# raulmur/ORB_SLAM2

Hardware: AMD Instinct MI355X
Metric: frames/s ORB extract+match, 1241x376 gray, 2000 kpts, 8 lvls (higher is better)
Workload: dtype u8

## Files before the change

### orb_slam2_amd/csrc/orbhip_kernels_extract.hip

```cpp
#include "orbhip_internal.h"
#include <type_traits>

#define WAVE 64

__device__ __forceinline__ bool xcd_frame_map(int nb, int nframes, int& tile, int& frame)
{
    const int id = blockIdx.x;
    if (nframes == 1) { tile = id; frame = 0; return true; }
    if (nframes < 8) { tile = id / nframes; frame = id - tile * nframes; return true; }
    const int j = id >> 3, fg = j / nb;
    tile = j - fg * nb; frame = fg * 8 + (id & 7);
    return frame < nframes;
}
static inline unsigned xcd_grid(int nb, int nframes) { return nframes < 8 ? (unsigned)nb * (unsigned)nframes : (unsigned)nb * 8u * (unsigned)((nframes + 7) / 8); }

typedef unsigned short pku16 __attribute__((vector_size(4)));
typedef short pki16 __attribute__((vector_size(4)));
typedef unsigned u32_unaligned __attribute__((aligned(1)));
#define ORBHIP_GLOBAL __attribute__((address_space(1)))
template <typename T> __device__ __forceinline__ ORBHIP_GLOBAL T* uniform_ptr(T* p)
{
    const unsigned long long a = (unsigned long long)p;
    const unsigned lo = (unsigned)__builtin_amdgcn_readfirstlane((int)(unsigned)a), hi = (unsigned)__builtin_amdgcn_readfirstlane((int)(unsigned)(a >> 32));
    return (ORBHIP_GLOBAL T*)(((unsigned long long)hi << 32) | lo);
// ... 263 lines not shown
    int tile, frame;
    if (!xcd_frame_map(gx * gyn, P.nframes, tile, frame)) return;
    frame += P.frame0;
    __shared__ unsigned s_t0[PYR_SROWS * PYR_SDW], s_t1[PYR_SROWS * PYR_SDW];
    const int tid = threadIdx.y * 64 + threadIdx.x, wv = __builtin_amdgcn_readfirstlane((int)threadIdx.y);
    const int tx = tile % gx;
    int ty = (tile / gx) * nt;
    const int tyend = min(ty + nt, gy);
    PyrStep st;
    st.S.src = level_src(P, frame, level - 1, st.S.spitch);
    st.T = pyr_dma_issue(P, g, tx, ty, tid, s_t0, st.S);
    const PyrGroup G = P.xgrp[g.xgrp_off + min(tx * (PYR_TW / 4) + (int)threadIdx.x, (g.w - 1) >> 2)];
    for (; ty < tyend; ty += 2) {
        pyr_step(P, g, tx, ty, tyend, frame, tid, threadIdx.x, wv, G, s_t0, s_t1, st);
        if (ty + 1 < tyend) pyr_step(P, g, tx, ty + 1, tyend, frame, tid, threadIdx.x, wv, G, s_t1, s_t0, st);
    }
}

__global__ __launch_bounds__(256) void k_pyramid_level_direct(ExtractParams P, int level)
{
    const LevelGeom g = P.geom[level];
    const int gx = (g.w + PYR_TW - 1) / PYR_TW, gy = (g.h + PYR_TH - 1) / PYR_TH;
    int tile, frame;
    if (!xcd_frame_map(gx * gy, P.nframes, tile, frame)) return;
    frame += P.frame0;
    const int x4 = (tile % gx) * PYR_TW + threadIdx.x * 4, ytop = (tile / gx) * PYR_TH + threadIdx.y * PYR_RPT;
    if (x4 >= g.w) return;
    int spitch; const uint8_t* src = level_src(P, frame, level - 1, spitch);
    pyr_rows(g, P.xtab + g.xtab_off, P.ytab + g.ytab_off, src, spitch, 0, x4, ytop, P.pyr + (long long)frame * P.plane_frame_bytes + g.plane_off + x4);
}

__device__ __forceinline__ int qt_wave_incl_scan(int v, int lane);
#define PC_T 256
#define PC_GIT 3
#define PC_YIT 2
#define PC_RIT 16
struct PcLevel { int w, src_h, pitch, plane_off, xgrp_off, ytab_off, goff, yoff, x0, x1, y0, y1; unsigned rcp; };
__global__ __launch_bounds__(PC_T) void k_pyramid_cascade(ExtractParams P)
{
    HIP_DYNAMIC_SHARED(unsigned char, pc_lds)
    __shared__ PcLevel s_lv[ORBHIP_MAX_LEVELS];
    int tile, frame;
    if (!xcd_frame_map(P.pc_ntx * P.pc_nty, P.nframes, tile, frame)) return;
    frame += P.frame0;
    const int tid = (int)threadIdx.x, L = P.nlevels;
    const int ty = tile / P.pc_ntx, tx = tile - ty * P.pc_ntx;
    if (tid < 64) {
        const int l = min(tid, L - 1);
        const LevelGeom g = P.geom[l];
        const short2 a = P.pc_xr[l * P.pc_ntx + tx], b = P.pc_yr[l * P.pc_nty + ty];
        const int ng = ((a.y - a.x) >> 2) + 1;
        const int nx = (tid >= 1 && tid < L) ? ng : 0, ny = (tid >= 1 && tid < L) ? b.y - b.x + 1 : 0;
        const int go = qt_wave_incl_scan(nx, tid) - nx, yo = qt_wave_incl_scan(ny, tid) - ny;
        if (tid < L) s_lv[tid] = PcLevel{g.w, g.src_h, g.pitch, g.plane_off, g.xgrp_off, g.ytab_off, go, yo, a.x, a.y, b.x, b.y, 0xffffffffu / (unsigned)ng + 1u};
        if (tid == L - 1) { s_lv[0].goff = go + nx; s_lv[0].yoff = yo + ny; }
    }
    __syncthreads();
    uint4* const s_grp = reinterpret_cast<uint4*>(pc_lds + P.pc_buf0 + P.pc_buf1);
    int2* const s_yt = reinterpret_cast<int2*>(s_grp + 3 * P.pc_xcap);
    {
        const int gtot = s_lv[0].goff, ytot = s_lv[0].yoff;
        int goffs[ORBHIP_MAX_LEVELS], yoffs[ORBHIP_MAX_LEVELS];
#pragma unroll
        for (int l = 0; l < ORBHIP_MAX_LEVELS; l++) { goffs[l] = s_lv[min(l, L - 1)].goff; yoffs[l] = s_lv[min(l, L - 1)].yoff; }
        uint4 gv[PC_GIT]; int2 yv[PC_YIT]; unsigned rv[PC_RIT];
#pragma unroll
        for (int k = 0; k < PC_GIT; k++) {
            const int i = min(tid + PC_T * k, 3 * gtot - 1), e = i / 3, piece = i - 3 * e;
            int l = 1;
#pragma unroll
            for (int q = 2; q < ORBHIP_MAX_LEVELS; q++) if (q < L && e >= goffs[q]) l = q;
            const PcLevel& v = s_lv[l];
            gv[k] = reinterpret_cast<const uint4*>(P.xgrp + v.xgrp_off + (v.x0 >> 2) + (e - v.goff))[piece];
        }
#pragma unroll
        for (int k = 0; k < PC_YIT; k++) {
            const int i = min(tid + PC_T * k, ytot - 1);
            int l = 1;
#pragma unroll
            for (int q = 2; q < ORBHIP_MAX_LEVELS; q++) if (q < L && i >= yoffs[q]) l = q;
            const PcLevel& v = s_lv[l];
            yv[k] = P.ytab[v.ytab_off + v.y0 + i - v.yoff];
        }
        const PcLevel R = s_lv[0];
        int spitch; const uint8_t* src = level_src(P, frame, 0, spitch);
        const int ng = ((R.x1 - R.x0) >> 2) + 1, n0 = ng * (R.y1 - R.y0 + 1);
#pragma unroll
        for (int k = 0; k < PC_RIT; k++) {
            const int i = min(tid + PC_T * k, n0 - 1);
            const int r = ng == 1 ? i : (int)__umulhi((unsigned)i, R.rcp), g4 = i - r * ng, x = R.x0 + 4 * g4;
            const uint8_t* p = src + (long long)(R.y0 + r) * spitch + x;
            unsigned w;
            if (x + 3 < R.w) w = *reinterpret_cast<const u32_unaligned*>(p);
            else { w = 0; for (int q = 0; q < 4; q++) if (x + q < R.w) w |= (unsigned)p[q] << (8 * q); }
            rv[k] = w;
        }
#pragma unroll
        for (int k = 0; k < PC_GIT; k++) if (tid + PC_T * k < 3 * gtot) s_grp[tid + PC_T * k] = gv[k];
#pragma unroll
        for (int k = 0; k < PC_YIT; k++) if (tid + PC_T * k < ytot) s_yt[tid + PC_T * k] = yv[k];
#pragma unroll
        for (int k = 0; k < PC_RIT; k++) if (tid + PC_T * k < n0) reinterpret_cast<unsigned*>(pc_lds)[tid + PC_T * k] = rv[k];
    }
    __syncthreads();
    for (int l = 1; l < L; l++) {
        const PcLevel R = s_lv[l], S = s_lv[l - 1];
        const int ng = ((R.x1 - R.x0) >> 2) + 1, rows = R.y1 - R.y0 + 1, spd = ((S.x1 - S.x0) >> 2) + 1;
        const unsigned* sb = reinterpret_cast<const unsigned*>(pc_lds + ((l & 1) ? 0 : P.pc_buf0));
        unsigned* db = reinterpret_cast<unsigned*>(pc_lds + ((l & 1) ? P.pc_buf0 : 0));
        const PyrGroup* grp = reinterpret_cast<const PyrGroup*>(s_grp) + R.goff; const int2* yt = s_yt + R.yoff;
        uint8_t* gdst = P.pyr + (long long)frame * P.plane_frame_bytes + R.plane_off;
        const bool keep = l + 1 < L;
        for (int i = tid; i < ng * rows; i += PC_T) {
            const int gy = ng == 1 ? i : (int)__umulhi((unsigned)i, R.rcp), g4 = i - gy * ng, y = R.y0 + gy, x4 = R.x0 + 4 * g4;
            const PyrGroup G = grp[g4];
            const int2 ye = yt[gy];
            const unsigned b0s = (unsigned)ye.y << 16, b1s = (unsigned)ye.y & 0xffff0000u;
            const int ra = min(max(ye.x, 0), R.src_h - 1) - S.y0, rb = min(max(ye.x + 1, 0), R.src_h - 1) - S.y0;
            const unsigned sh = (unsigned)G.sx0 & 3u;
            const unsigned* colp = sb + ((G.sx0 - S.x0) >> 2);
            unsigned h0[4], h1[4];
            pyr_hrow(colp + ra * spd, sh, G, h0);
            pyr_hrow(colp + rb * spd, sh, G, h1);
            unsigned out = 0;
#pragma unroll
            for (int k = 0; k < 4; k++) out |= ((__umulhi(b0s, h0[k]) + __umulhi(b1s, h1[k]) + 2u) >> 2) << (8 * k);
            out &= x4 + 4 <= R.w ? 0xffffffffu : (0xffffffffu >> (8 * (x4 + 4 - R.w)));
            if (keep) db[i] = out;
            *reinterpret_cast<unsigned*>(gdst + (long long)y * R.pitch + x4) = out;
        }
        lds_barrier();
    }
}
void orbhip_launch_pyramid_cascade(const ExtractParams& P, int nframes, hipStream_t s)
{
    ExtractParams Q = P; Q.nframes = nframes;
    const size_t lds = (size_t)P.pc_buf0 + P.pc_buf1 + (size_t)P.pc_xcap * sizeof(PyrGroup) + (size_t)P.pc_ycap * sizeof(int2);
    hipLaunchKernelGGL(k_pyramid_cascade, dim3(xcd_grid(P.pc_ntx * P.pc_nty, nframes), 1, 1), dim3(PC_T, 1, 1), lds, s, Q);
}

bool orbhip_pyramid_tile_fits(int src_cols_per_tile, int src_rows_per_tile) { return ((src_cols_per_tile + 3) >> 2) + 1 <= PYR_SDW && src_rows_per_tile <= PYR_SROWS; }
int orbhip_pyramid_tile_dwords() { return PYR_SDW; }
int orbhip_blur_mfma_tile_w() { return BM_COLS * BM_BLOCKS; }
int orbhip_blur_mfma_tile_h() { return BM_ROWS; }
int orbhip_pyramid_tile_w() { return PYR_TW; }
int orbhip_pyramid_tile_h() { return PYR_TH; }

void orbhip_launch_pyramid_level(const ExtractParams& P, int level, int w, int h, int mode, int nframes, hipStream_t s)
{
    ExtractParams Q = P; Q.nframes = nframes;
    dim3 grid(xcd_grid(((w + PYR_TW - 1) / PYR_TW) * ((h + PYR_TH - 1) / PYR_TH), nframes), 1, 1), block(64, 4, 1);
    static const int nt_env = getenv("ORBHIP_PYR_NT") ? atoi(getenv("ORBHIP_PYR_NT")) : 0;
    const int nt = nt_env > 0 ? nt_env : nframes >= 384 ? 4 : nframes <= 8 ? 1 : 2;
    const int gyn = (((h + PYR_TH - 1) / PYR_TH) + nt - 1) / nt;
    if (mode == 2) hipLaunchKernelGGL(k_pyramid_level_g, dim3(xcd_grid(((w + PYR_TW - 1) / PYR_TW) * gyn, nframes), 1, 1), block, 0, s, Q, level, nt);
    else if (mode == 1) hipLaunchKernelGGL(k_pyramid_level, grid, block, 0, s, Q, level);
    else hipLaunchKernelGGL(k_pyramid_level_direct, grid, block, 0, s, Q, level);
}

struct GrayParams {
    const uint8_t* src; long long src_frame_stride; int src_row_stride;
    uint8_t* dst; long long dst_frame_stride; int dst_pitch;
    int w, h, channels, k0, k2;
};
__device__ __forceinline__ uint32_t gray14(uint32_t c0, uint32_t c1, uint32_t c2, int k0, int k2)
{
    return (c0 * (uint32_t)k0 + c1 * 9617u + c2 * (uint32_t)k2 + 8192u) >> 14;
}
__global__ __launch_bounds__(256) void k_to_gray(GrayParams G)
{
    const int x = (blockIdx.x * 256 + threadIdx.x) * 4, y = blockIdx.y, f = blockIdx.z;
    if (x >= G.w) return;
    const uint8_t* srow = G.src + (long long)f * G.src_frame_stride + (long long)y * G.src_row_stride + (long long)x * G.channels;
    uint8_t* drow = G.dst + (long long)f * G.dst_frame_stride + (long long)y * G.dst_pitch + x;
    const bool whole = x + 4 <= G.w, aligned = (((uintptr_t)srow) & 3) == 0;
    if (whole && aligned) {
        const uint32_t* s4 = (const uint32_t*)srow;
        uint32_t g0, g1, g2, g3;
        if (G.channels == 3) {
            const uint32_t a = s4[0], b = s4[1], c = s4[2];
            g0 = gray14(a & 255, (a >> 8) & 255, (a >> 16) & 255, G.k0, G.k2);
            g1 = gray14(a >> 24, b & 255, (b >> 8) & 255, G.k0, G.k2);
            g2 = gray14((b >> 16) & 255, b >> 24, c & 255, G.k0, G.k2);
            g3 = gray14((c >> 8) & 255, (c >> 16) & 255, c >> 24, G.k0, G.k2);
        } else {
            const uint32_t a = s4[0], b = s4[1], c = s4[2], d = s4[3];
            g0 = gray14(a & 255, (a >> 8) & 255, (a >> 16) & 255, G.k0, G.k2);
            g1 = gray14(b & 255, (b >> 8) & 255, (b >> 16) & 255, G.k0, G.k2);
            g2 = gray14(c & 255, (c >> 8) & 255, (c >> 16) & 255, G.k0, G.k2);
            g3 = gray14(d & 255, (d >> 8) & 255, (d >> 16) & 255, G.k0, G.k2);
        }
        *(uint32_t*)drow = g0 | (g1 << 8) | (g2 << 16) | (g3 << 24);
    } else {
        const int n = min(4, G.w - x);
        for (int i = 0; i < n; i++) {
            const uint8_t* p = srow + i * G.channels;
            drow[i] = (uint8_t)gray14(p[0], p[1], p[2], G.k0, G.k2);
        }
    }
}
void orbhip_launch_to_gray(const uint8_t* src, long long src_frame_stride, int src_row_stride, uint8_t* dst, long long dst_frame_stride,
                           int dst_pitch, int w, int h, int channels, bool rgb_order, int nframes, hipStream_t s)
{
    GrayParams G{src, src_frame_stride, src_row_stride, dst, dst_frame_stride, dst_pitch, w, h, channels,
                 rgb_order ? 4899 : 1868, rgb_order ? 1868 : 4899};
    dim3 grid((w + 1023) / 1024, h, nframes), block(256, 1, 1);
    hipLaunchKernelGGL(k_to_gray, grid, block, 0, s, G);
}

#define BLUR_TW 128
#define BLUR_TH 32
#define BLUR_SROW 144
__device__ __forceinline__ int reflect101_clamped(int p, int len)
{
    if (p < 0) p = -p; else if (p >= len) p = 2 * (len - 1) - p;
    return min(max(p, 0), len - 1);
}
struct BlurK { float k0, k1, k2, k3; unsigned dot_lo, dot_hi; };
#define BLUR_SDW (BLUR_SROW / 4)
#define BLUR_SROWS (BLUR_TH + 6)
__global__ __launch_bounds__(256) void k_blur(ExtractParams P, BlurK K)
{
    int tile, frame;
    if (!xcd_frame_map(P.nblur_tiles, P.nframes, tile, frame)) return;
    frame += P.frame0;
    const TileDesc t = P.blur_tiles[tile];
    const int tid = threadIdx.x;
    const LevelGeom g = P.geom[t.level];
    int spitch; const uint8_t* src = level_src(P, frame, t.level, spitch);
    __shared__ unsigned s_src[BLUR_SROWS * BLUR_SDW];
    __shared__ float4 s_h[BLUR_SROWS * (BLUR_TW / 4)];
    const bool aligned = ((((unsigned long long)src) | (unsigned long long)spitch) & 3ull) == 0;
    {
        const int wave = __builtin_amdgcn_readfirstlane(tid >> 6), lane = tid & 63;
        const int gx = t.x0 - 4 + 4 * lane;
        const bool act = lane < 34, edge = act && !(aligned && gx >= 0 && gx + 3 < g.w);
        unsigned v[10];
#pragma unroll
        for (int j = 0; j < 10; j++) {
            const uint8_t* row = src + (long long)reflect101_clamped(t.y0 - 3 + wave + 4 * j, g.h) * spitch + (t.x0 - 4);
            v[j] = (act && !edge) ? *reinterpret_cast<const unsigned*>(row + (unsigned)(4 * lane)) : 0u;
        }
        if (edge) {
            const int x0r = reflect101_clamped(gx, g.w), x1r = reflect101_clamped(gx + 1, g.w), x2r = reflect101_clamped(gx + 2, g.w), x3r = reflect101_clamped(gx + 3, g.w);
#pragma unroll
            for (int j = 0; j < 10; j++) {
                const uint8_t* row = src + (long long)reflect101_clamped(t.y0 - 3 + wave + 4 * j, g.h) * spitch;
                v[j] = (unsigned)row[x0r] | ((unsigned)row[x1r] << 8) | ((unsigned)row[x2r] << 16) | ((unsigned)row[x3r] << 24);
            }
        }
#pragma unroll
        for (int j = 0; j < 10; j++) {
            const int r = wave + 4 * j;
            if (act && r < BLUR_SROWS) s_src[r * BLUR_SDW + lane] = v[j];
        }
    }
    __syncthreads();
    for (int i = tid; i < BLUR_SROWS * 32; i += 256) {
        const int r = i >> 5, q = i & 31;
        const unsigned* p = &s_src[r * BLUR_SDW + q];
        const unsigned w0 = p[0], w1 = p[1], w2 = p[2];
        float4 o;
        o.x = (float)__builtin_amdgcn_udot4(__builtin_amdgcn_alignbyte(w1, w0, 1), K.dot_lo, __builtin_amdgcn_udot4(__builtin_amdgcn_alignbyte(w2, w1, 1), K.dot_hi, 0u, false), false);
        o.y = (float)__builtin_amdgcn_udot4(__builtin_amdgcn_alignbyte(w1, w0, 2), K.dot_lo, __builtin_amdgcn_udot4(__builtin_amdgcn_alignbyte(w2, w1, 2), K.dot_hi, 0u, false), false);
        o.z = (float)__builtin_amdgcn_udot4(__builtin_amdgcn_alignbyte(w1, w0, 3), K.dot_lo, __builtin_amdgcn_udot4(__builtin_amdgcn_alignbyte(w2, w1, 3), K.dot_hi, 0u, false), false);
        o.w = (float)__builtin_amdgcn_udot4(w1, K.dot_lo, __builtin_amdgcn_udot4(w2, K.dot_hi, 0u, false), false);
        s_h[r * (BLUR_TW / 4) + q] = o;
    }
    __syncthreads();
    const int q = tid & 31, rg = tid >> 5;
    const int gx = t.x0 + 4 * q;
    if (gx >= g.w) return;
    float h[10][4];
#pragma unroll
    for (int r = 0; r < 10; r++) { const float4 v = s_h[(4 * rg + r) * (BLUR_TW / 4) + q]; h[r][0] = v.x; h[r][1] = v.y; h[r][2] = v.z; h[r][3] = v.w; }
    const bool half_even = P.blur_round_mode == 1 && gx < (g.w & ~3);
    uint8_t* dstbase = P.blur + (long long)frame * P.plane_frame_bytes + g.plane_off + gx;
    auto strip = [&](auto he) {
#pragma unroll
        for (int r = 0; r < 4; r++) {
            const int gy = t.y0 + 4 * rg + r;
            if (gy >= g.h) break;
            unsigned out = 0;
#pragma unroll
            for (int k = 0; k < 4; k++) {
                float sum = K.k0 * h[r + 3][k];
                sum = __builtin_fmaf(K.k1, h[r + 2][k] + h[r + 4][k], sum);
                sum = __builtin_fmaf(K.k2, h[r + 1][k] + h[r + 5][k], sum);
                sum = __builtin_fmaf(K.k3, h[r][k] + h[r + 6][k], sum);
                const float v = decltype(he)::value ? sum * (1.0f / 65536.0f) : __builtin_floorf(__builtin_fmaf(sum, 1.0f / 65536.0f, 0.5f));
                out = __builtin_amdgcn_cvt_pk_u8_f32(v, (unsigned)k, out);
            }
            *reinterpret_cast<unsigned*>(dstbase + (long long)gy * g.pitch) = out;
        }
    };
    if (half_even) strip(std::true_type{}); else strip(std::false_type{});
}

typedef int v4i __attribute__((vector_size(16)));
typedef int v2i __attribute__((vector_size(8)));
typedef int v16i __attribute__((vector_size(64)));
#define BM_IN_DW 68
#define BM_OUT_DW 57
struct BlurTile { TileDesc t; LevelGeom g; const uint8_t* src; int spitch; };
__device__ __forceinline__ BlurTile blur_tile(const ExtractParams& P, int frame, int tile)
{
    BlurTile T; T.t = P.blur_tiles[tile]; T.g = P.geom[T.t.level]; T.src = level_src(P, frame, T.t.level, T.spitch);
    return T;
}
__device__ __forceinline__ void blur_issue(const BlurTile& T, int wave, int lane, unsigned* s_in)
{
    const LevelGeom& g = T.g; const int x0 = T.t.x0, y0 = T.t.y0, spitch = T.spitch; const uint8_t* src = T.src;
    const int w4 = g.w & ~3;
    const int c0 = x0 - 4 + 4 * lane;
    const unsigned coff = (unsigned)min(max(c0, 0), w4 - 4);
#pragma unroll
    for (int r = 0; r < 8; r++) {
        const int row = 8 * wave + r;
        const ORBHIP_GLOBAL uint8_t* rp = uniform_ptr(src + (long long)reflect101_clamped(y0 - 3 + row, g.h) * spitch);
        lds_dma_dword(rp + coff, reinterpret_cast<uint8_t*>(s_in + row * BM_IN_DW));
    }
}
__device__ __forceinline__ void blur_fix(const BlurTile& T, int wave, int lane, unsigned* s_in)
{
    const LevelGeom& g = T.g; const int x0 = T.t.x0, y0 = T.t.y0, spitch = T.spitch; const uint8_t* src = T.src;
    const int w4 = g.w & ~3;
    const bool fix_left = x0 == 0, fix_right = x0 + 252 > w4;
    if (fix_left || fix_right) {
        const int rr = lane >> 3, slot = lane & 7, row = 8 * wave + rr;
        const int cfix = slot == 0 ? -4 : w4 + 4 * (slot - 1);
        const int dw = (cfix - (x0 - 4)) >> 2;
        const bool act = (slot == 0 ? fix_left : (slot <= 2 && fix_right)) && dw >= 0 && dw < 64;
        if (act) {
            const uint8_t* rowp = src + (long long)reflect101_clamped(y0 - 3 + row, g.h) * spitch;
            unsigned wv = 0;
#pragma unroll
            for (int b = 0; b < 4; b++) wv |= (unsigned)rowp[reflect101_clamped(cfix + b, g.w)] << (8 * b);
            s_in[row * BM_IN_DW + dw] = wv;
        }
    }
}
__device__ __forceinline__ void blur_compute(const ExtractParams& P, const BlurTile& T, int wave, int lane, const unsigned* s_in, unsigned* s_out, const unsigned* s_band)
{
    const LevelGeom& g = T.g; const int x0 = T.t.x0;
    const int w4 = g.w & ~3;
    const int i = lane & 31, h = lane >> 5;
    const v4i HB1 = *reinterpret_cast<const v4i*>(s_band + 4 * lane), HB2 = *reinterpret_cast<const v4i*>(s_band + 256 + 4 * lane), VB = *reinterpret_cast<const v4i*>(s_band + 512 + 4 * lane);
    const v16i zero = {0, 0, 0, 0, 0, 0, 0, 0, 0, 0, 0, 0, 0, 0, 0, 0};
    const int he_limit = P.blur_round_mode == 1 ? w4 : 0;
    const float kbias = (float)(257 * 128 * 257) * (1.0f / 65536.0f);
#pragma unroll 1
    for (int c = wave; c < BM_BLOCKS; c += 4) {
        const int xb = x0 + 32 * c;
        if (xb >= g.w) break;
        v4i A1 = *reinterpret_cast<const v4i*>(s_in + i * BM_IN_DW + 8 * c + 4 * h);
        const v2i a2 = *reinterpret_cast<const v2i*>(s_in + i * BM_IN_DW + 8 * c + 8);
        v4i A2 = {a2[0], a2[1], 0, 0};
#pragma unroll
        for (int d = 0; d < 4; d++) { A1[d] ^= (int)0x80808080u; A2[d] ^= (int)0x80808080u; }
        v16i acc = __builtin_amdgcn_mfma_i32_32x32x32_i8(A1, HB1, zero, 0, 0, 0);
        acc = __builtin_amdgcn_mfma_i32_32x32x32_i8(A2, HB2, acc, 0, 0, 0);
        v4i Alo, Ahi;
#pragma unroll
        for (int gq = 0; gq < 4; gq++) {
            const unsigned r0 = (unsigned)acc[4 * gq] + 128u * 257u, r1 = (unsigned)acc[4 * gq + 1] + 128u * 257u;
            const unsigned r2 = (unsigned)acc[4 * gq + 2] + 128u * 257u, r3 = (unsigned)acc[4 * gq + 3] + 128u * 257u;
            const unsigned t01 = __builtin_amdgcn_perm(r1, r0, 0x05010400u);
            const unsigned t23 = __builtin_amdgcn_perm(r3, r2, 0x05010400u);
            Alo[gq] = (int)(__builtin_amdgcn_perm(t23, t01, 0x05040100u) ^ 0x80808080u);
            Ahi[gq] = (int)(__builtin_amdgcn_perm(t23, t01, 0x07060302u) ^ 0x80808080u);
        }
        const v16i clo = __builtin_amdgcn_mfma_i32_32x32x32_i8(Alo, VB, zero, 0, 0, 0);
        const v16i chi = __builtin_amdgcn_mfma_i32_32x32x32_i8(Ahi, VB, zero, 0, 0, 0);
        if (i < BM_ROWS) {
            const bool all_he = xb + 32 <= he_limit, none_he = xb >= he_limit;
            auto finish = [&](auto mode) {
#pragma unroll
                for (int gq = 0; gq < 4; gq++) {
                    const int gx = xb + 8 * gq + 4 * h;
                    unsigned out = 0;
#pragma unroll
                    for (int k = 0; k < 4; k++) {
                        const float raw = (float)((chi[4 * gq + k] << 8) + clo[4 * gq + k]);
                        const float q = __builtin_fmaf(raw, 1.0f / 65536.0f, kbias);
                        float v;
                        if (decltype(mode)::value == 1) v = q;
                        else if (decltype(mode)::value == 0) v = __builtin_floorf(q + 0.5f);
                        else v = gx < he_limit ? q : __builtin_floorf(q + 0.5f);
                        out = __builtin_amdgcn_cvt_pk_u8_f32(v, (unsigned)k, out);
                    }
                    s_out[i * BM_OUT_DW + 8 * c + 2 * gq + h] = out;
                }
            };
            if (all_he) finish(std::integral_constant<int, 1>{}); else if (none_he) finish(std::integral_constant<int, 0>{}); else finish(std::integral_constant<int, 2>{});
        }
    }
}
__device__ __forceinline__ void blur_store(const ExtractParams& P, const BlurTile& T, int frame, int wave, int lane, const unsigned* s_out)
{
    const LevelGeom& g = T.g; const int x0 = T.t.x0, y0 = T.t.y0;
    uint8_t* dst = P.blur + (long long)frame * P.plane_frame_bytes + g.plane_off;
    const int gx = x0 + 4 * lane;
    if (lane < 8 * BM_BLOCKS && gx < g.w)
        for (int r = wave; r < BM_ROWS && y0 + r < g.h; r += 4)
            *reinterpret_cast<unsigned*>(dst + (long long)(y0 + r) * g.pitch + gx) = s_out[r * BM_OUT_DW + lane];
}

__device__ __forceinline__ void blur_mfma_tile(const ExtractParams& P, int tile, int frame, unsigned* s_in, unsigned* s_out, unsigned* s_band)
{
#pragma unroll
    for (int k = 0; k < 3; k++) s_band[256 * k + threadIdx.x] = reinterpret_cast<const unsigned*>(P.blur_band)[256 * k + threadIdx.x];
    const int wave = __builtin_amdgcn_readfirstlane(threadIdx.x >> 6), lane = threadIdx.x & 63;
    const BlurTile T = blur_tile(P, frame, tile);
    blur_issue(T, wave, lane, s_in);
    lds_dma_wait();
    __builtin_amdgcn_wave_barrier();
    blur_fix(T, wave, lane, s_in);
    __syncthreads();
    blur_compute(P, T, wave, lane, s_in, s_out, s_band);
    __syncthreads();
    blur_store(P, T, frame, wave, lane, s_out);
}
__global__ __launch_bounds__(256, 5) void k_blur_mfma(ExtractParams P)
{
    __shared__ __attribute__((aligned(16))) unsigned s_in[32 * BM_IN_DW];
    __shared__ unsigned s_out[BM_ROWS * BM_OUT_DW];
    __shared__ __attribute__((aligned(16))) unsigned s_band[3 * 64 * 4];
    int tile, frame;
    if (!xcd_frame_map(P.nblur_tiles, P.nframes, tile, frame)) return;
    blur_mfma_tile(P, tile, frame + P.frame0, s_in, s_out, s_band);
}

void orbhip_launch_blur(const ExtractParams& P, const int gk[4], int nframes, hipStream_t s, int tile0, int ntiles)
{
    BlurK K; K.k0 = (float)gk[0]; K.k1 = (float)gk[1]; K.k2 = (float)gk[2]; K.k3 = (float)gk[3];
    K.dot_lo = (unsigned)gk[3] | ((unsigned)gk[2] << 8) | ((unsigned)gk[1] << 16) | ((unsigned)gk[0] << 24);
    K.dot_hi = (unsigned)gk[1] | ((unsigned)gk[2] << 8) | ((unsigned)gk[3] << 16);
    ExtractParams Q = P; Q.nframes = nframes;
    if (ntiles >= 0) { Q.blur_tiles = P.blur_tiles + tile0; Q.nblur_tiles = ntiles; }
    if (Q.nblur_tiles <= 0) return;
    if (P.blur_band) hipLaunchKernelGGL(k_blur_mfma, dim3(xcd_grid(Q.nblur_tiles, nframes), 1, 1), dim3(256, 1, 1), 0, s, Q);
    else hipLaunchKernelGGL(k_blur, dim3(xcd_grid(Q.nblur_tiles, nframes), 1, 1), dim3(256, 1, 1), 0, s, Q, K);
}

#define FC_WAVES 4

__device__ __forceinline__ pku16 pmin(pku16 a, pku16 b) { return a < b ? a : b; }
__device__ __forceinline__ pku16 pmax(pku16 a, pku16 b) { return a > b ? a : b; }

template <int I> __device__ __forceinline__ pku16 row_pair(unsigned w0, unsigned w1, unsigned w2)
{
    unsigned r;
    if (I <= 6) r = __builtin_amdgcn_perm(w1, w0, 0x0c000c00u | (unsigned)I | ((unsigned)(I + 1) << 16));
    else r = __builtin_amdgcn_perm(w2, w1, 0x0c000c00u | (unsigned)(I - 4) | ((unsigned)(I - 3) << 16));
    return (pku16)r;
}

__device__ __forceinline__ pki16 fast_score_pair(const pku16 r[16], pku16 c)
{
    pku16 m = pmin(r[0], r[8]);
#pragma unroll
    for (int k = 1; k < 8; k++) m = pmax(m, pmin(r[k], r[k + 8]));
    const pki16 nb = ~(((pki16)c - (pki16)m) >> 15);
    const pku16 cm = (pku16)nb & (pku16){0x00ff, 0x00ff};
    pku16 q[16], pn[16], sn[16];
#pragma unroll
    for (int i = 0; i < 16; i++) q[i] = r[i] ^ cm;
#pragma unroll
    for (int b = 0; b < 16; b += 8) {
        pn[b] = q[b]; sn[b + 7] = q[b + 7];
#pragma unroll
        for (int i = 1; i < 8; i++) { pn[b + i] = pmin(pn[b + i - 1], q[b + i]); sn[b + 7 - i] = pmin(sn[b + 8 - i], q[b + 7 - i]); }
    }
    pku16 hi = pmin(sn[0], pn[8]);
#pragma unroll
    for (int i = 1; i < 16; i++) hi = pmax(hi, pmin(sn[i], pn[(i + 8) & 15]));
    const pki16 one = {1, 1};
    return (pki16)hi - (pki16)(c ^ cm) - one;
}

__host__ __device__ __forceinline__ int fc_wave_bytes(int pbytes, int sstride, int srows, int listcap)
{
    return ((pbytes + 15) & ~15) + ((sstride * srows + 4 + 15) & ~15) + ((2 * listcap + 15) & ~15);
}

__device__ __forceinline__ pku16 row_pair_v(unsigned lo, unsigned hi, unsigned sel) { return (pku16)__builtin_amdgcn_perm(hi, lo, sel); }
#define FC_RING_V(s) { \
    row_pair_v(w[6][0], w[6][1], s[3]), row_pair_v(w[6][0], w[6][1], s[4]), row_pair_v(w[5][1], w[5][2], s[1]), row_pair_v(w[4][1], w[4][2], s[2]), \
    row_pair_v(w[3][1], w[3][2], s[2]), row_pair_v(w[2][1], w[2][2], s[2]), row_pair_v(w[1][1], w[1][2], s[1]), row_pair_v(w[0][0], w[0][1], s[4]), \
    row_pair_v(w[0][0], w[0][1], s[3]), row_pair_v(w[0][0], w[0][1], s[2]), row_pair_v(w[1][0], w[1][1], s[1]), row_pair_v(w[2][0], w[2][1], s[0]), \
    row_pair_v(w[3][0], w[3][1], s[0]), row_pair_v(w[4][0], w[4][1], s[0]), row_pair_v(w[5][0], w[5][1], s[1]), row_pair_v(w[6][0], w[6][1], s[2]) }
#define FC_RING(Q) { \
    row_pair<3 + Q + 0>(w[6][0], w[6][1], w[6][2]), row_pair<3 + Q + 1>(w[6][0], w[6][1], w[6][2]), row_pair<3 + Q + 2>(w[5][0], w[5][1], w[5][2]), row_pair<3 + Q + 3>(w[4][0], w[4][1], w[4][2]), \
    row_pair<3 + Q + 3>(w[3][0], w[3][1], w[3][2]), row_pair<3 + Q + 3>(w[2][0], w[2][1], w[2][2]), row_pair<3 + Q + 2>(w[1][0], w[1][1], w[1][2]), row_pair<3 + Q + 1>(w[0][0], w[0][1], w[0][2]), \
    row_pair<3 + Q + 0>(w[0][0], w[0][1], w[0][2]), row_pair<3 + Q - 1>(w[0][0], w[0][1], w[0][2]), row_pair<3 + Q - 2>(w[1][0], w[1][1], w[1][2]), row_pair<3 + Q - 3>(w[2][0], w[2][1], w[2][2]), \
    row_pair<3 + Q - 3>(w[3][0], w[3][1], w[3][2]), row_pair<3 + Q - 3>(w[4][0], w[4][1], w[4][2]), row_pair<3 + Q - 2>(w[5][0], w[5][1], w[5][2]), row_pair<3 + Q - 1>(w[6][0], w[6][1], w[6][2]) }

__device__ __forceinline__ pku16 psubsat(pku16 a, pku16 b) { return __builtin_elementwise_sub_sat(a, b); }
__device__ __forceinline__ unsigned fast_pretest_pair(const pku16 r[16], pku16 c, pku16 tt)
{
    pku16 mn = pmax(r[0], r[8]), mx = pmin(r[0], r[8]);
#pragma unroll
    for (int k = 2; k < 8; k += 2) { mn = pmin(mn, pmax(r[k], r[k + 8])); mx = pmax(mx, pmin(r[k], r[k + 8])); }
    return (unsigned)(psubsat(mn, c + tt) | psubsat(psubsat(c, tt), mx));
}

__device__ __forceinline__ int fc_rank(unsigned long long m, int base)
{
    return (int)__builtin_amdgcn_mbcnt_hi((unsigned)(m >> 32), __builtin_amdgcn_mbcnt_lo((unsigned)m, (unsigned)base));
}

__device__ __forceinline__ void fc_load_window(const uint8_t* patch, int PS, int y, int grp, unsigned (&w)[7][3])
{
    const unsigned* prow = reinterpret_cast<const unsigned*>(patch + y * PS) + grp;
#pragma unroll
    for (int r = 0; r < 7; r++) { w[r][0] = prow[r * (PS >> 2)]; w[r][1] = prow[r * (PS >> 2) + 1]; w[r][2] = prow[r * (PS >> 2) + 2]; }
}

template <int CPS, int CSS>
__global__ __launch_bounds__(256, 8) void k_fast_cells(ExtractParams P)
{
    HIP_DYNAMIC_SHARED(unsigned, fc_lds)
    const int wave = __builtin_amdgcn_readfirstlane(threadIdx.x >> 6), lane = threadIdx.x & 63;
    int tile, frame;
    if (!xcd_frame_map((P.fc_ncells + FC_WAVES - 1) / FC_WAVES, P.nframes, tile, frame)) return;
    frame += P.frame0;
    const int cell_last = P.fc_cell0 + P.fc_ncells - 1;
    const bool have = P.fc_cell0 + tile * FC_WAVES + wave <= cell_last;
    const int cell_id = min(P.fc_cell0 + tile * FC_WAVES + wave, cell_last);
    const CellDesc cd = P.cells[cell_id];
    const int pw = cd.maxX - cd.iniX, ph = cd.maxY - cd.iniY;
    const int cw = pw - 6, ch = ph - 6;
    const bool work = have && !cd.skipped && cw > 0 && ch > 0;
    const int PS = CPS ? CPS : P.fc_pstride, SS = CSS ? CSS : P.fc_sstride;
    const int WB = fc_wave_bytes(P.fc_pbytes, SS, P.fc_srows, P.fc_listcap);
    const int score_off = (P.fc_pbytes + 15) & ~15, list_off = score_off + ((SS * P.fc_srows + 4 + 15) & ~15);
    uint8_t* const lds0 = reinterpret_cast<uint8_t*>(fc_lds);
    uint8_t* wbase = lds0 + wave * WB;
    uint8_t* patch = wbase;
    uint8_t* score = wbase + score_off;
    unsigned short* list = reinterpret_cast<unsigned short*>(wbase + list_off);
    int* const sh = reinterpret_cast<int*>(lds0 + FC_WAVES * WB);
    const int ng = (cw + 3) >> 2;
    if (lane == 0) sh[4 + wave] = cw;
    if (work) {
        int spitch; const uint8_t* src = level_src(P, frame, cd.level, spitch);
        src += (long long)cd.iniY * spitch + cd.iniX;
        const ORBHIP_GLOBAL uint8_t* gp = uniform_ptr(src);
        const unsigned maxoff = (unsigned)((ph - 1) * spitch + 4 * (((pw + 3) >> 2) - 1));
        const int np = P.fc_np;
        for (int k0 = 0; k0 < np; k0 += 8) {
            const int4* tab = P.fc_dma + (k0 >> 1) * 64 + lane;
            int4 rr[2], dd[2];
#pragma unroll
            for (int j = 0; j < 2; j++) if (k0 + 4 * j < np) { rr[j] = tab[(2 * j) * 64]; dd[j] = tab[(2 * j + 1) * 64]; }
#pragma unroll
            for (int j = 0; j < 2; j++) if (k0 + 4 * j < np) {
                const int r4[4] = {rr[j].x, rr[j].y, rr[j].z, rr[j].w}, d4[4] = {dd[j].x, dd[j].y, dd[j].z, dd[j].w};
#pragma unroll
                for (int q = 0; q < 4; q++) if (k0 + 4 * j + q < np)
                    lds_dma_dword(gp + min(__umul24((unsigned)r4[q], (unsigned)spitch) + (unsigned)d4[q], maxoff), patch + (k0 + 4 * j + q) * 256);
            }
        }
        for (int i = lane; i < ((SS >> 2) * (ch + 2) + 1 + 3) >> 2; i += 64) reinterpret_cast<uint4*>(score)[i] = uint4{0u, 0u, 0u, 0u};
        lds_dma_wait();
    }
    __builtin_amdgcn_wave_barrier();
    const int rp = (64 * cd.inv_ng) >> 16;
    const int sr = (lane * cd.inv_ng) >> 16, grp = lane - sr * ng;
    const bool lane_ok = sr < rp;
    const unsigned long long lok_mask = __builtin_amdgcn_ballot_w64(lane_ok);
    unsigned* out = P.cell_cand + (long long)frame * P.cand_slots_per_frame + cd.cand_idx;

    int count = 0;
    bool busy = work;
    for (int phase = 0; phase < 2; phase++) {
        const int th = phase ? P.minTh : P.iniTh;
        const pku16 tt = {(unsigned short)th, (unsigned short)th};
        int nq = 0;
        if (busy)
        for (int yb = 0; yb < ch; yb += rp) {
            const int yy = yb + sr, y = min(yy, ch - 1);
            const bool act = lane_ok && yy < ch;
            unsigned pa, pb;
            {
                unsigned w[7][3];
                fc_load_window(patch, PS, y, grp, w);
                const pku16 ra[16] = FC_RING(0);
                const pku16 rb[16] = FC_RING(2);
                pa = fast_pretest_pair(ra, row_pair<3>(w[3][0], w[3][1], w[3][2]), tt);
                pb = fast_pretest_pair(rb, row_pair<5>(w[3][0], w[3][1], w[3][2]), tt);
            }
            const unsigned long long am = __builtin_amdgcn_ballot_w64(yy < ch) & lok_mask;
            const unsigned long long ma = __builtin_amdgcn_ballot_w64(pa != 0) & am, mb = __builtin_amdgcn_ballot_w64(pb != 0) & am;
            const bool la = act && pa != 0, lb = act && pb != 0;
            int pos = fc_rank(mb, fc_rank(ma, nq));
            if (la) list[pos++] = (unsigned short)((y << 8) | (2 * grp));
            if (lb) list[pos] = (unsigned short)((y << 8) | (2 * grp + 1));
            nq += __popcll(ma) + __popcll(mb);
        }
        if (lane == 0) sh[wave] = nq;
        __syncthreads();
        {
            const int o1 = __builtin_amdgcn_readfirstlane(sh[0]), o2 = o1 + __builtin_amdgcn_readfirstlane(sh[1]), o3 = o2 + __builtin_amdgcn_readfirstlane(sh[2]);
            const int T = o3 + __builtin_amdgcn_readfirstlane(sh[3]);
            const int rot = (tile ^ (tile >> 2) ^ (tile >> 5) ^ (tile >> 7) ^ frame) & (FC_WAVES - 1);
            for (int e0 = 64 * ((wave - rot) & (FC_WAVES - 1)); e0 < T; e0 += 64 * FC_WAVES) {
                const int e = e0 + lane;
                if (e < T) {
                    const int d1 = e - o1, d2 = e - o2, d3 = e - o3;
                    const int le = (int)min(min((unsigned)e, (unsigned)d1), min((unsigned)d2, (unsigned)d3));
                    const int j = 3 + (d1 >> 31) + (d2 >> 31) + (d3 >> 31);
                    const int jo = (int)__umul24((unsigned)j, (unsigned)WB);
                    const int cwj = sh[4 + j];
                    const uint8_t* jb = lds0 + jo;
                    const int id = *reinterpret_cast<const unsigned short*>(lds0 + jo + list_off + 2 * le), y = id >> 8, pr = id & 0xff, x0 = 2 * pr;
                    const unsigned* prow = reinterpret_cast<const unsigned*>(jb + y * PS) + (pr >> 1);
                    const unsigned shsel = (pr & 1) ? 0x00020002u : 0u;
                    const unsigned sel[5] = {0x0c010c00u + shsel, 0x0c020c01u + shsel, 0x0c030c02u + shsel, 0x0c040c03u + shsel, 0x0c050c04u + shsel};
                    unsigned w[7][3];
#pragma unroll
                    for (int r = 0; r < 7; r++) { w[r][0] = prow[r * (PS >> 2)]; w[r][1] = prow[r * (PS >> 2) + 1]; w[r][2] = prow[r * (PS >> 2) + 2]; }
                    const pku16 ra[16] = FC_RING_V(sel);
                    const pki16 sa = fast_score_pair(ra, row_pair_v(w[3][0], w[3][1], sel[3]));
                    int s0 = sa[0], s1 = sa[1];
                    if (s0 < th || x0 >= cwj) s0 = 0;
                    if (s1 < th || x0 + 1 >= cwj) s1 = 0;
                    *reinterpret_cast<unsigned short*>(lds0 + jo + score_off + (y + 1) * SS + 4 + x0) = (unsigned short)(s0 | (s1 << 8));
                }
            }
        }
        __syncthreads();
        if (busy)
        for (int qb = 0; qb < nq; qb += 64) {
            unsigned gtm = 0, rbm = 0; int y = 0, x0 = 0;
            if (qb + lane < nq) {
                int li = qb + lane;
                asm volatile("" : "+v"(li));
                const int id = list[li];
                y = id >> 8; x0 = 2 * (id & 0xff);
                const int qo = (y + 1) * SS + 4 + x0 - 1;
                const unsigned* qa = reinterpret_cast<const unsigned*>(score) + (qo >> 2);
                const unsigned shb = (unsigned)qo & 3u;
                const int sdw = SS >> 2;
                const unsigned ra4 = __builtin_amdgcn_alignbyte(qa[1 - sdw], qa[-sdw], shb);
                const unsigned rb4 = __builtin_amdgcn_alignbyte(qa[1], qa[0], shb);
                const unsigned rc4 = __builtin_amdgcn_alignbyte(qa[1 + sdw], qa[sdw], shb);
                auto bp = [](unsigned r, unsigned sel) { return (pku16)__builtin_amdgcn_perm(0u, r, sel); };
                const pku16 cpair = bp(rb4, 0x0c020c01u);
                pku16 nb = pmax(bp(rb4, 0x0c010c00u), bp(rb4, 0x0c030c02u));
                nb = pmax(nb, pmax(bp(ra4, 0x0c010c00u), pmax(bp(ra4, 0x0c020c01u), bp(ra4, 0x0c030c02u))));
                nb = pmax(nb, pmax(bp(rc4, 0x0c010c00u), pmax(bp(rc4, 0x0c020c01u), bp(rc4, 0x0c030c02u))));
                gtm = (unsigned)psubsat(cpair, nb); rbm = rb4;
            }
            const bool keep[2] = {(gtm & 0xffffu) != 0, (gtm >> 16) != 0};
            const int scv[2] = {(int)(rbm >> 8) & 0xff, (int)(rbm >> 16) & 0xff};
            const unsigned long long m0 = __builtin_amdgcn_ballot_w64(keep[0]), m1 = __builtin_amdgcn_ballot_w64(keep[1]);
            int rank = fc_rank(m1, fc_rank(m0, count));
#pragma unroll
            for (int q = 0; q < 2; q++)
                if (keep[q]) {
                    const unsigned px = (unsigned)(x0 + q + 3 + cd.shiftX), py = (unsigned)(y + 3 + cd.shiftY);
                    if (rank < cd.cand_cap) out[rank] = px | (py << 12) | ((unsigned)scv[q] << 24);
                    rank++;
                }
            count += __popcll(m0) + __popcll(m1);
        }
        if (count > 0) busy = false;
        if (phase == 0 && busy) for (int i = lane; i < ((SS >> 2) * (ch + 2) + 1 + 3) >> 2; i += 64) reinterpret_cast<uint4*>(score)[i] = uint4{0u, 0u, 0u, 0u};
    }
    if (have && lane == 0) P.cell_count[(long long)frame * P.ncells_total + cell_id] = work ? min(count, cd.cand_cap) : 0;
}
#undef FC_RING
#undef FC_RING_V

void orbhip_launch_fast_cells(const ExtractParams& P, int nframes, hipStream_t s, int cell0, int ncells)
{
    const size_t lds = (size_t)FC_WAVES * fc_wave_bytes(P.fc_pbytes, P.fc_sstride, P.fc_srows, P.fc_listcap) + 32;
    ExtractParams Q = P; Q.nframes = nframes;
    Q.fc_cell0 = ncells < 0 ? 0 : cell0; Q.fc_ncells = ncells < 0 ? P.ncells_total : ncells;
    if (Q.fc_ncells <= 0) return;
    const dim3 grid(xcd_grid((Q.fc_ncells + FC_WAVES - 1) / FC_WAVES, nframes), 1, 1);
    if (Q.fc_pstride == 48 && Q.fc_sstride == 36) hipLaunchKernelGGL((k_fast_cells<48, 36>), grid, dim3(256, 1, 1), lds, s, Q);
    else hipLaunchKernelGGL((k_fast_cells<0, 0>), grid, dim3(256, 1, 1), lds, s, Q);
}

#define QT_T 256

__device__ __forceinline__ int qt_digit(unsigned code, int depth)
{
    return depth < ORBHIP_QT_DEPTH ? (int)((code >> (2 * (ORBHIP_QT_DEPTH - 1 - depth))) & 3u) : 0;
}

__device__ __forceinline__ int qt_wave_incl_scan(int v, int lane)
{
    (void)lane;
    int t = v + __builtin_amdgcn_update_dpp(0, v, 0x111, 0xf, 0xf, true);
    t += __builtin_amdgcn_update_dpp(0, v, 0x112, 0xf, 0xf, true);
    t += __builtin_amdgcn_update_dpp(0, v, 0x113, 0xf, 0xf, true);
    t += __builtin_amdgcn_update_dpp(0, t, 0x114, 0xf, 0xe, true);
    t += __builtin_amdgcn_update_dpp(0, t, 0x118, 0xf, 0xc, true);
    t += __builtin_amdgcn_update_dpp(0, t, 0x142, 0xa, 0xf, true);
    t += __builtin_amdgcn_update_dpp(0, t, 0x143, 0xc, 0xf, true);
    return t;
}
template <bool TRAILING_BARRIER = true>
__device__ __forceinline__ int qt_block_exscan(int* a, int n, int* scratch, int tid)
{
    const int lane = tid & 63, wave = tid >> 6, nch = (n + 63) >> 6;
    for (int c = wave; c < nch; c += QT_T / 64) {
        const int i = c * 64 + lane, v = i < n ? a[i] : 0;
        const int incl = qt_wave_incl_scan(v, lane);
        if (i < n) a[i] = incl - v;
        if (lane == 63) scratch[c] = incl;
    }
    __syncthreads();
    if (wave == 0) {
        int run = 0;
        for (int cb = 0; cb < nch; cb += 64) {
            const int v = (cb + lane < nch) ? scratch[cb + lane] : 0;
            const int incl = qt_wave_incl_scan(v, lane);
            if (cb + lane < nch) scratch[cb + lane] = run + incl - v;
            run += __shfl(incl, 63);
        }
        if (lane == 0) scratch[-1] = run;
    }
    __syncthreads();
    for (int i = tid; i < n; i += QT_T) a[i] += scratch[i >> 6];
    const int total = scratch[-1];
    if (TRAILING_BARRIER) __syncthreads();
    return total;
}

#define QT_KPT 16
#define QT_REGKEYS (QT_KPT * QT_T)

int orbhip_quadtree_scr(int maxn, int maxcells) { return (std::max(maxn, maxcells) + 63) / 64 + 2; }
size_t orbhip_quadtree_lds_bytes(int maxn, int maxcells)
{
    const size_t ints = (size_t)maxn * (2 + 4) + (size_t)std::max(2 * maxcells + 1, 5 * maxn) + orbhip_quadtree_scr(maxn, maxcells) + 16;
    return sizeof(int) * ints + (size_t)maxn * 4 * 2 + (((size_t)maxn * 2 + 3) & ~(size_t)3);
}

struct QtKeysReg {
// ... 623 lines not shown
```

Measured before the change: 201,900.

## Process multiple blur tiles per block with prefetch of next tile's input

The MFMA blur kernel now loops over four tiles per workgroup. It issues the LDS DMA for the next tile's input rows before storing the current tile's output, and keeps the band matrices in registers instead of LDS. Border fixup now reads the reflected bytes from LDS rather than global memory. Tile and geometry descriptors come through scalar loads, and the LDS accesses are written as explicit asm. This amortises per-block setup and overlaps global loads with stores, but it launches four times fewer blocks, which reduces parallelism and adds hazards around reusing the same LDS buffers.

Measured after the change: 203,400 (median of 6 runs). Within noise of the previous version (+0.7%).

```diff
diff --git a/orb_slam2_amd/csrc/orbhip_kernels_extract.hip b/orb_slam2_amd/csrc/orbhip_kernels_extract.hip
--- a/orb_slam2_amd/csrc/orbhip_kernels_extract.hip
+++ b/orb_slam2_amd/csrc/orbhip_kernels_extract.hip
@@ -589,59 +589,99 @@
 typedef int v16i __attribute__((vector_size(64)));
 #define BM_IN_DW 68
 #define BM_OUT_DW 57
-struct BlurTile { TileDesc t; LevelGeom g; const uint8_t* src; int spitch; };
+__device__ __forceinline__ unsigned lds_addr(const void* p) { return (unsigned)(unsigned long long)(orbhip_lptr)p; }
+__device__ __forceinline__ unsigned lds_read4_u8(const uint8_t* p0, const uint8_t* p1, const uint8_t* p2, const uint8_t* p3)
+{
+#if defined(__HIP_DEVICE_COMPILE__) && __HIP_DEVICE_COMPILE__
+    unsigned b0, b1, b2, b3;
+    asm volatile("ds_read_u8 %0, %4\n\tds_read_u8 %1, %5\n\tds_read_u8 %2, %6\n\tds_read_u8 %3, %7\n\ts_waitcnt lgkmcnt(0)"
+                 : "=&v"(b0), "=&v"(b1), "=&v"(b2), "=&v"(b3) : "v"(lds_addr(p0)), "v"(lds_addr(p1)), "v"(lds_addr(p2)), "v"(lds_addr(p3)));
+    return b0 | (b1 << 8) | (b2 << 16) | (b3 << 24);
+#else
+    return (unsigned)*p0 | ((unsigned)*p1 << 8) | ((unsigned)*p2 << 16) | ((unsigned)*p3 << 24);
+#endif
+}
+__device__ __forceinline__ unsigned lds_read_b32(const unsigned* p)
+{
+#if defined(__HIP_DEVICE_COMPILE__) && __HIP_DEVICE_COMPILE__
+    unsigned v;
+    asm volatile("ds_read_b32 %0, %1\n\ts_waitcnt lgkmcnt(0)" : "=&v"(v) : "v"(lds_addr(p)));
+    return v;
+#else
+    return *p;
+#endif
+}
+__device__ __forceinline__ void lds_write_b32(unsigned* p, unsigned v)
+{
+#if defined(__HIP_DEVICE_COMPILE__) && __HIP_DEVICE_COMPILE__
+    asm volatile("ds_write_b32 %0, %1" :: "v"(lds_addr(p)), "v"(v) : "memory");
+#else
+    *p = v;
+#endif
+}
+__device__ __forceinline__ void lds_read_a(const unsigned* p16, const unsigned* p8, v4i& a1, v2i& a2)
+{
+#if defined(__HIP_DEVICE_COMPILE__) && __HIP_DEVICE_COMPILE__
+    asm volatile("ds_read_b128 %0, %2\n\tds_read_b64 %1, %3\n\ts_waitcnt lgkmcnt(0)" : "=&v"(a1), "=&v"(a2) : "v"(lds_addr(p16)), "v"(lds_addr(p8)));
+#else
+    a1 = *reinterpret_cast<const v4i*>(p16); a2 = *reinterpret_cast<const v2i*>(p8);
+#endif
+}
+struct BlurTile { int x0, y0, w, h, pitch, plane_off; const uint8_t* src; int spitch; };
 __device__ __forceinline__ BlurTile blur_tile(const ExtractParams& P, int frame, int tile)
 {
-    BlurTile T; T.t = P.blur_tiles[tile]; T.g = P.geom[T.t.level]; T.src = level_src(P, frame, T.t.level, T.spitch);
+    const unsigned long long d = scalar_load(reinterpret_cast<const unsigned long long*>(P.blur_tiles + tile));
+    const int level = (int)(d & 0xffff);
+    BlurTile T; T.x0 = (int)((d >> 16) & 0xffff); T.y0 = (int)((d >> 32) & 0xffff);
+    const LevelGeom* g = P.geom + level;
+    T.w = scalar_load(&g->w); T.h = scalar_load(&g->h); T.pitch = scalar_load(&g->pitch); T.plane_off = scalar_load(&g->plane_off);
+    if (level == 0) { T.spitch = P.img0_pitch; T.src = P.img0 + (long long)frame * P.img0_frame_stride; }
+    else { T.spitch = T.pitch; T.src = P.pyr + (long long)frame * P.plane_frame_bytes + T.plane_off; }
     return T;
 }
 __device__ __forceinline__ void blur_issue(const BlurTile& T, int wave, int lane, unsigned* s_in)
 {
-    const LevelGeom& g = T.g; const int x0 = T.t.x0, y0 = T.t.y0, spitch = T.spitch; const uint8_t* src = T.src;
-    const int w4 = g.w & ~3;
-    const int c0 = x0 - 4 + 4 * lane;
-    const unsigned coff = (unsigned)min(max(c0, 0), w4 - 4);
+    const unsigned coff = (unsigned)min(max(T.x0 - 4 + 4 * lane, 0), T.w - 4);
 #pragma unroll
     for (int r = 0; r < 8; r++) {
         const int row = 8 * wave + r;
-        const ORBHIP_GLOBAL uint8_t* rp = uniform_ptr(src + (long long)reflect101_clamped(y0 - 3 + row, g.h) * spitch);
+        const ORBHIP_GLOBAL uint8_t* rp = uniform_ptr(T.src + (long long)reflect101_clamped(T.y0 - 3 + row, T.h) * T.spitch);
         lds_dma_dword(rp + coff, reinterpret_cast<uint8_t*>(s_in + row * BM_IN_DW));
     }
 }
 __device__ __forceinline__ void blur_fix(const BlurTile& T, int wave, int lane, unsigned* s_in)
 {
-    const LevelGeom& g = T.g; const int x0 = T.t.x0, y0 = T.t.y0, spitch = T.spitch; const uint8_t* src = T.src;
-    const int w4 = g.w & ~3;
-    const bool fix_left = x0 == 0, fix_right = x0 + 252 > w4;
-    if (fix_left || fix_right) {
-        const int rr = lane >> 3, slot = lane & 7, row = 8 * wave + rr;
-        const int cfix = slot == 0 ? -4 : w4 + 4 * (slot - 1);
-        const int dw = (cfix - (x0 - 4)) >> 2;
-        const bool act = (slot == 0 ? fix_left : (slot <= 2 && fix_right)) && dw >= 0 && dw < 64;
-        if (act) {
-            const uint8_t* rowp = src + (long long)reflect101_clamped(y0 - 3 + row, g.h) * spitch;
-            unsigned wv = 0;
-#pragma unroll
-            for (int b = 0; b < 4; b++) wv |= (unsigned)rowp[reflect101_clamped(cfix + b, g.w)] << (8 * b);
-            s_in[row * BM_IN_DW + dw] = wv;
-        }
-    }
-}
-__device__ __forceinline__ void blur_compute(const ExtractParams& P, const BlurTile& T, int wave, int lane, const unsigned* s_in, unsigned* s_out, const unsigned* s_band)
-{
-    const LevelGeom& g = T.g; const int x0 = T.t.x0;
-    const int w4 = g.w & ~3;
+    const int w = T.w, w4 = w & ~3, sxa = T.x0 - 4, dr = (w4 - sxa) >> 2;
+    const bool left = T.x0 == 0, right = dr < 64;
+    if (!left && !right) return;
+    const int slot = lane & 3, d = slot == 0 ? 0 : dr + slot - 1;
+    const bool act = lane < 32 && (slot == 0 ? left : slot <= 2 && right && d < 64);
+    uint8_t* row = reinterpret_cast<uint8_t*>(s_in + (8 * wave + (lane >> 2)) * BM_IN_DW);
+    const uint8_t* src[4];
+#pragma unroll
+    for (int b = 0; b < 4; b++) {
+        const int sc = reflect101_clamped(sxa + 4 * d + b, w);
+        src[b] = row + (sc < w4 ? sc - sxa : 4 * dr + sc - (w - 4));
+    }
+    const unsigned v = act ? lds_read4_u8(src[0], src[1], src[2], src[3]) : 0u;
+    __builtin_amdgcn_wave_barrier();
+    if (act) lds_write_b32(reinterpret_cast<unsigned*>(row) + d, v);
+}
+__device__ __forceinline__ void blur_compute(const ExtractParams& P, const BlurTile& T, int wave, int lane, const unsigned* s_in, unsigned* s_out, const v4i (&band)[3])
+{
+    const int x0 = T.x0;
+    const int w4 = T.w & ~3;
     const int i = lane & 31, h = lane >> 5;
-    const v4i HB1 = *reinterpret_cast<const v4i*>(s_band + 4 * lane), HB2 = *reinterpret_cast<const v4i*>(s_band + 256 + 4 * lane), VB = *reinterpret_cast<const v4i*>(s_band + 512 + 4 * lane);
+    const v4i HB1 = band[0], HB2 = band[1], VB = band[2];
     const v16i zero = {0, 0, 0, 0, 0, 0, 0, 0, 0, 0, 0, 0, 0, 0, 0, 0};
     const int he_limit = P.blur_round_mode == 1 ? w4 : 0;
     const float kbias = (float)(257 * 128 * 257) * (1.0f / 65536.0f);
 #pragma unroll 1
     for (int c = wave; c < BM_BLOCKS; c += 4) {
         const int xb = x0 + 32 * c;
-        if (xb >= g.w) break;
-        v4i A1 = *reinterpret_cast<const v4i*>(s_in + i * BM_IN_DW + 8 * c + 4 * h);
-        const v2i a2 = *reinterpret_cast<const v2i*>(s_in + i * BM_IN_DW + 8 * c + 8);
+        if (xb >= T.w) break;
+        v4i A1; v2i a2;
+        lds_read_a(s_in + i * BM_IN_DW + 8 * c + 4 * h, s_in + i * BM_IN_DW + 8 * c + 8, A1, a2);
         v4i A2 = {a2[0], a2[1], 0, 0};
 #pragma unroll
         for (int d = 0; d < 4; d++) { A1[d] ^= (int)0x80808080u; A2[d] ^= (int)0x80808080u; }
@@ -676,21 +716,25 @@
                         else v = gx < he_limit ? q : __builtin_floorf(q + 0.5f);
                         out = __builtin_amdgcn_cvt_pk_u8_f32(v, (unsigned)k, out);
                     }
-                    s_out[i * BM_OUT_DW + 8 * c + 2 * gq + h] = out;
+                    lds_write_b32(s_out + i * BM_OUT_DW + 8 * c + 2 * gq + h, out);
                 }
             };
             if (all_he) finish(std::integral_constant<int, 1>{}); else if (none_he) finish(std::integral_constant<int, 0>{}); else finish(std::integral_constant<int, 2>{});
         }
     }
+#if defined(__HIP_DEVICE_COMPILE__) && __HIP_DEVICE_COMPILE__
+    asm volatile("s_waitcnt lgkmcnt(0)" ::: "memory");
+#endif
 }
 __device__ __forceinline__ void blur_store(const ExtractParams& P, const BlurTile& T, int frame, int wave, int lane, const unsigned* s_out)
 {
-    const LevelGeom& g = T.g; const int x0 = T.t.x0, y0 = T.t.y0;
-    uint8_t* dst = P.blur + (long long)frame * P.plane_frame_bytes + g.plane_off;
-    const int gx = x0 + 4 * lane;
-    if (lane < 8 * BM_BLOCKS && gx < g.w)
-        for (int r = wave; r < BM_ROWS && y0 + r < g.h; r += 4)
-            *reinterpret_cast<unsigned*>(dst + (long long)(y0 + r) * g.pitch + gx) = s_out[r * BM_OUT_DW + lane];
+    uint8_t* dst = P.blur + (long long)frame * P.plane_frame_bytes + T.plane_off;
+    const int gx = T.x0 + 4 * lane, ld = min(lane, 8 * BM_BLOCKS - 1);
+    for (int r = wave; r < BM_ROWS && T.y0 + r < T.h; r += 4) {
+        const unsigned v = lds_read_b32(s_out + r * BM_OUT_DW + ld);
+        if (lane < 8 * BM_BLOCKS && gx < T.w)
+            *reinterpret_cast<unsigned*>(dst + (long long)(T.y0 + r) * T.pitch + gx) = v;
+    }
 }
 
 __device__ __forceinline__ void blur_mfma_tile(const ExtractParams& P, int tile, int frame, unsigned* s_in, unsigned* s_out, unsigned* s_band)
@@ -703,19 +747,42 @@
     lds_dma_wait();
     __builtin_amdgcn_wave_barrier();
     blur_fix(T, wave, lane, s_in);
-    __syncthreads();
-    blur_compute(P, T, wave, lane, s_in, s_out, s_band);
+    lds_barrier_spelled();
+    const v4i band[3] = {*reinterpret_cast<const v4i*>(s_band + 4 * lane), *reinterpret_cast<const v4i*>(s_band + 256 + 4 * lane), *reinterpret_cast<const v4i*>(s_band + 512 + 4 * lane)};
+    blur_compute(P, T, wave, lane, s_in, s_out, band);
     __syncthreads();
     blur_store(P, T, frame, wave, lane, s_out);
 }
+#define BM_NT 4
 __global__ __launch_bounds__(256, 5) void k_blur_mfma(ExtractParams P)
 {
     __shared__ __attribute__((aligned(16))) unsigned s_in[32 * BM_IN_DW];
     __shared__ unsigned s_out[BM_ROWS * BM_OUT_DW];
-    __shared__ __attribute__((aligned(16))) unsigned s_band[3 * 64 * 4];
-    int tile, frame;
-    if (!xcd_frame_map(P.nblur_tiles, P.nframes, tile, frame)) return;
-    blur_mfma_tile(P, tile, frame + P.frame0, s_in, s_out, s_band);
+    int grp, frame;
+    if (!xcd_frame_map((P.nblur_tiles + BM_NT - 1) / BM_NT, P.nframes, grp, frame)) return;
+    frame += P.frame0;
+    const int wave = __builtin_amdgcn_readfirstlane(threadIdx.x >> 6), lane = threadIdx.x & 63;
+    int t = grp * BM_NT;
+    const int tend = min(t + BM_NT, P.nblur_tiles);
+    BlurTile T = blur_tile(P, frame, t);
+    blur_issue(T, wave, lane, s_in);
+    v4i band[3];
+#pragma unroll
+    for (int k = 0; k < 3; k++) band[k] = reinterpret_cast<const v4i*>(P.blur_band)[64 * k + lane];
+    for (;;) {
+        lds_dma_wait();
+        __builtin_amdgcn_wave_barrier();
+        blur_fix(T, wave, lane, s_in);
+        lds_barrier_spelled();
+        blur_compute(P, T, wave, lane, s_in, s_out, band);
+        lds_barrier_spelled();
+        const bool more = ++t < tend;
+        BlurTile N = T;
+        if (more) { N = blur_tile(P, frame, t); blur_issue(N, wave, lane, s_in); }
+        blur_store(P, T, frame, wave, lane, s_out);
+        if (!more) break;
+        T = N;
+    }
 }
 
 void orbhip_launch_blur(const ExtractParams& P, const int gk[4], int nframes, hipStream_t s, int tile0, int ntiles)
@@ -726,7 +793,7 @@
     ExtractParams Q = P; Q.nframes = nframes;
     if (ntiles >= 0) { Q.blur_tiles = P.blur_tiles + tile0; Q.nblur_tiles = ntiles; }
     if (Q.nblur_tiles <= 0) return;
-    if (P.blur_band) hipLaunchKernelGGL(k_blur_mfma, dim3(xcd_grid(Q.nblur_tiles, nframes), 1, 1), dim3(256, 1, 1), 0, s, Q);
+    if (P.blur_band) hipLaunchKernelGGL(k_blur_mfma, dim3(xcd_grid((Q.nblur_tiles + BM_NT - 1) / BM_NT, nframes), 1, 1), dim3(256, 1, 1), 0, s, Q);
     else hipLaunchKernelGGL(k_blur, dim3(xcd_grid(Q.nblur_tiles, nframes), 1, 1), dim3(256, 1, 1), 0, s, Q, K);
 }
 
```
